# lucian-ilie/SAGE2

Measured on NVIDIA B200. Metric: reads/sec through exact-overlap graph build (SAGE2 steps 1-3), higher is better.
Workload: dtype u64

## Files before the change

sage2_b200/csrc/core.cuh:

```cuda
#pragma once
#include <stdint.h>

#if defined(__CUDACC__)
#define SG_HD __host__ __device__ __forceinline__
#else
#define SG_HD inline
#endif

namespace sg {

typedef uint64_t u64;
typedef uint32_t u32;

constexpr int kMaxWords = 32;
constexpr int kHashThreshold = 100;
constexpr u32 kConnectionsLimit = 300;

SG_HD int words_for_len(int max_len) { return (2 * max_len + 16 + 63) / 64; }
SG_HD int storage_words(int SW) { return SW <= 4 ? 4 : (SW <= 8 ? 8 : (SW <= 16 ? 16 : 32)); }
SG_HD int rec_len(const u64 *rec, int SW) { return (int)(rec[SW - 1] & 0xFFFFull); }
SG_HD int hash_len_for(int min_overlap) { return min_overlap > 64 ? 64 : min_overlap; }

SG_HD u64 window32(const u64 *X, int SW, int s)
{
// ... 26 lines not shown
    return true;
}

SG_HD u64 rev2(u64 w)
{
#if defined(__CUDA_ARCH__)
    w = __brevll(w);
    return ((w >> 1) & 0x5555555555555555ull) | ((w & 0x5555555555555555ull) << 1);
#else
    w = ((w >> 2) & 0x3333333333333333ull) | ((w & 0x3333333333333333ull) << 2);
    w = ((w >> 4) & 0x0F0F0F0F0F0F0F0Full) | ((w & 0x0F0F0F0F0F0F0F0Full) << 4);
    return __builtin_bswap64(w);
#endif
}

SG_HD void revcomp_record(const u64 *F, u64 *R, int SW, int len)
{
    const int sh = 64 * SW - 2 * len;
    const int q = sh >> 6, r = sh & 63;
    for (int w = 0; w < SW; ++w) {
        const int i0 = w + q, i1 = w + q + 1;
        const u64 a = i0 < SW ? rev2(~F[SW - 1 - i0]) : 0ull;
        const u64 b = i1 < SW ? rev2(~F[SW - 1 - i1]) : 0ull;
        R[w] = r == 0 ? a : ((a << r) | (b >> (64 - r)));
    }
    R[SW - 1] |= (u64)len;
}

SG_HD u64 mix64(u64 x)
{
    x ^= x >> 33; x *= 0xff51afd7ed558ccdull; x ^= x >> 33; x *= 0xc4ceb9fe1a85ec53ull; x ^= x >> 33;
    return x;
}
SG_HD u64 hash_key(u64 v0, u64 v1) { return mix64(v1 ^ mix64(v0 + 0x9e3779b97f4a7c15ull)); }
SG_HD u64 mulhi64(u64 a, u64 b)
{
#if defined(__CUDA_ARCH__)
    return __umul64hi(a, b);
#else
    return (u64)(((unsigned __int128)a * b) >> 64);
#endif
// ... 152 lines not shown
```

sage2_b200/csrc/device_utils.cuh:

```cuda
#pragma once
#include <cuda_runtime.h>
#include <stdint.h>
#include <stdio.h>
#include <algorithm>
#include <stdexcept>
#include <string>
#include <vector>

namespace sg {

typedef uint64_t u64;
typedef uint32_t u32;

struct CudaError : public std::runtime_error {
    explicit CudaError(const std::string &m) : std::runtime_error(m) {}
};

#define SG_CUDA(call)                                                                           \
    do {                                                                                        \
        cudaError_t e__ = (call);                                                               \
        if (e__ != cudaSuccess)                                                                 \
            throw sg::CudaError(std::string(#call) + " failed: " + cudaGetErrorString(e__) +    \
                                " at " + __FILE__ + ":" + std::to_string(__LINE__));            \
    } while (0)
// ... 128 lines not shown
{
    cudaStreamSynchronize(st);
    cudaMemPool_t pool;
    if (cudaDeviceGetDefaultMemPool(&pool, device) == cudaSuccess) cudaMemPoolTrimTo(pool, 0);
}

constexpr int kSMs = 148;

inline unsigned long long &launch_counter() { static unsigned long long n = 0; return n; }
#define SG_LAUNCHED()                     \
    do {                                  \
        ++sg::launch_counter();           \
        SG_CUDA(cudaGetLastError());      \
    } while (0)

inline unsigned grid_for(u64 n, unsigned block, unsigned per_thread = 1)
{
    u64 g = (n + (u64)block * per_thread - 1) / ((u64)block * per_thread);
    if (g == 0) g = 1;
    SG_CHECK(g < 0x7FFFFFFFull, "grid too large");
    return (unsigned)g;
}

void exclusive_scan_u32(const u32 *in, u32 *out, u64 n, u32 *d_total, cudaStream_t st);

void reduce_or_and_u64(const u64 *keys, u64 n, u64 *d_or_and, cudaStream_t st);

struct SortCols {
    u64 *a[2];
    u64 *b[2];
// ... 10 lines not shown
```

sage2_b200/csrc/reads.cu:

```cuda
#include <stdlib.h>
#include "context.h"

namespace sg {

constexpr int K1_WARPS = 8;

__global__ void __launch_bounds__(K1_WARPS * 32) max_len_kernel(const int64_t *__restrict__ off, u64 n, int *out)
{
    int m = 0;
    for (u64 i = (u64)blockIdx.x * blockDim.x + threadIdx.x; i < n; i += (u64)gridDim.x * blockDim.x) {
        const int64_t d = off[i + 1] - off[i];
        const int l = d > 0x7FFFFFFF ? 0x7FFFFFFF : (int)d;
        m = l > m ? l : m;
    }
    m = __reduce_max_sync(0xffffffffu, m);
    if ((threadIdx.x & 31) == 0) atomicMax(out, m);
}

__global__ void __launch_bounds__(K1_WARPS * 32) pack_kernel(const uint8_t *__restrict__ bases, const int64_t *__restrict__ off,
                                                              u64 n, int k, int SW, u64 *__restrict__ rec,
                                                              unsigned long long *counters )
{
    __shared__ __align__(16) uint8_t sB[K1_WARPS][32 * kMaxWords];
    __shared__ u64 sF[K1_WARPS][kMaxWords], sR[K1_WARPS][kMaxWords];
// ... 278 lines not shown
    c.cnt.total_bp = h_cnt[1];
    c.cnt.avg_len = h_cnt[0] ? h_cnt[1] / h_cnt[0] : 0;
}

__global__ void iota_kernel(u32 *v, u64 n)
{
    for (u64 i = (u64)blockIdx.x * blockDim.x + threadIdx.x; i < n; i += (u64)gridDim.x * blockDim.x) v[i] = (u32)i;
}

__global__ void gather_word_kernel(const u64 *__restrict__ rec, const u32 *__restrict__ perm, u64 n, int SW, int w, u64 *__restrict__ key)
{
    for (u64 i = (u64)blockIdx.x * blockDim.x + threadIdx.x; i < n; i += (u64)gridDim.x * blockDim.x)
        key[i] = rec[(u64)perm[i] * SW + w];
}

__global__ void unique_flag_kernel(const u64 *__restrict__ rec, const u32 *__restrict__ perm, u64 n_good, int SW, u32 *__restrict__ flag)
{
    for (u64 i = (u64)blockIdx.x * blockDim.x + threadIdx.x; i < n_good; i += (u64)gridDim.x * blockDim.x) {
        u32 f = 1;
        if (i > 0) {
            const u64 *a = rec + (u64)perm[i] * SW, *b = rec + (u64)perm[i - 1] * SW;
            f = 0;
            for (int w = 0; w < SW; ++w) f |= (a[w] != b[w]);
        }
        flag[i] = f;
    }
}

template <bool WITH_RC>
__global__ void unique_write_kernel(const u64 *__restrict__ rec, const u32 *__restrict__ perm, const u32 *__restrict__ flag,
                                    const u32 *__restrict__ uidx, u64 n_good, int SW, int SWS,
                                    u64 *__restrict__ F, u64 *__restrict__ RC, uint16_t *__restrict__ len, u32 *__restrict__ start)
{
    for (u64 i = (u64)blockIdx.x * blockDim.x + threadIdx.x; i < n_good; i += (u64)gridDim.x * blockDim.x) {
        if (!flag[i]) continue;
        const u32 u = uidx[i];
        const u64 *a = rec + (u64)perm[i] * SW;
        u64 f[kMaxWords], r[kMaxWords];
        for (int w = 0; w < SW; ++w) f[w] = a[w];
        const int l = rec_len(f, SW);
        if (WITH_RC) revcomp_record(f, r, SW, l);
        for (int w = 0; w < SWS; ++w) { F[(u64)u * SWS + w] = w < SW ? f[w] : 0ull; if (WITH_RC) RC[(u64)u * SWS + w] = w < SW ? r[w] : 0ull; }
        len[u] = (uint16_t)l;
        start[u] = (u32)i;
    }
}

__global__ void freq_kernel(const u32 *__restrict__ start, u64 U, u64 n_good, uint16_t *__restrict__ freq)
{
    for (u64 u = (u64)blockIdx.x * blockDim.x + threadIdx.x; u < U; u += (u64)gridDim.x * blockDim.x) {
        const u64 e = (u + 1 < U) ? start[u + 1] : n_good;
        freq[u] = (uint16_t)(e - start[u]);
    }
}

static unsigned big_grid(u64 n, unsigned block = 256)
{
    unsigned g = grid_for(n, block, 4);
    return g > kSMs * 16u ? kSMs * 16u : g;
// ... 16 lines not shown
static int sort_skip_bits(u64 n)
{
    int lg = 0;
    while (lg < 63 && (1ull << lg) < n) ++lg;
    int bits = ((lg + 5 + 7) / 8) * 8;
    if (bits < 32) bits = 32;
    if (bits > 48) bits = 48;
    return 64 - bits;
}
__device__ __forceinline__ bool rec_less(const u64 *a, const u64 *b, int SW)
{
    for (int w = 0; w < SW; ++w) { const u64 x = a[w], y = b[w]; if (x != y) return x < y; }
    return false;
}
__global__ void __launch_bounds__(256) tie_fix_kernel(const u64 *__restrict__ rec, const u64 *__restrict__ key, u32 *__restrict__ perm, u64 n, int SW,
                                                        int kSortSkipBits, u32 *__restrict__ overflow)
{
    for (u64 i = (u64)blockIdx.x * blockDim.x + threadIdx.x; i < n; i += (u64)gridDim.x * blockDim.x) {
        const u64 k = key[i] >> kSortSkipBits;
        if ((i > 0 && (key[i - 1] >> kSortSkipBits) == k) || i + 1 >= n || (key[i + 1] >> kSortSkipBits) != k) continue;
        u64 e = i + 2;
        while (e < n && (key[e] >> kSortSkipBits) == k && e - i <= (u64)kTieLimit) ++e;
        if (e - i > (u64)kTieLimit) { *overflow = 1u; continue; }
        for (u64 a = i + 1; a < e; ++a) {
            const u32 x = perm[a];
            const u64 *rx = rec + (u64)x * SW;
            u64 b = a;
            while (b > i && rec_less(rx, rec + (u64)perm[b - 1] * SW, SW)) { perm[b] = perm[b - 1]; --b; }
            perm[b] = x;
        }
    }
}

__global__ void __launch_bounds__(256) run_boundary_kernel(const u64 *__restrict__ key, u64 n, int kSortSkipBits, u32 *__restrict__ flag)
{
    for (u64 i = (u64)blockIdx.x * blockDim.x + threadIdx.x; i < n; i += (u64)gridDim.x * blockDim.x)
        flag[i] = (i == 0 || (key[i] >> kSortSkipBits) != (key[i - 1] >> kSortSkipBits)) ? 1u : 0u;
}
__global__ void __launch_bounds__(256) run_count_kernel(const u32 *__restrict__ flag, const u32 *__restrict__ excl, u64 n, u32 *__restrict__ cnt)
{
    for (u64 i = (u64)blockIdx.x * blockDim.x + threadIdx.x; i < n; i += (u64)gridDim.x * blockDim.x)
        atomicAdd(&cnt[excl[i] + flag[i] - 1], 1u);
}
__global__ void __launch_bounds__(256) run_long_flag_kernel(const u32 *__restrict__ flag, const u32 *__restrict__ excl, const u32 *__restrict__ cnt, u64 n,
                                                            u32 *__restrict__ lflag)
{
    for (u64 i = (u64)blockIdx.x * blockDim.x + threadIdx.x; i < n; i += (u64)gridDim.x * blockDim.x)
        lflag[i] = cnt[excl[i] + flag[i] - 1] > (u32)kTieLimit ? 1u : 0u;
}
__global__ void __launch_bounds__(256) run_compact_kernel(const u32 *__restrict__ lflag, const u32 *__restrict__ lidx, const u32 *__restrict__ flag,
                                                          const u32 *__restrict__ excl, const u32 *__restrict__ perm, u64 n,
                                                          u32 *__restrict__ pos, u32 *__restrict__ val, u64 *__restrict__ run)
{
    for (u64 i = (u64)blockIdx.x * blockDim.x + threadIdx.x; i < n; i += (u64)gridDim.x * blockDim.x)
        if (lflag[i]) { const u32 j = lidx[i]; pos[j] = (u32)i; val[j] = perm[i]; run[j] = (u64)(excl[i] + flag[i] - 1); }
}
__global__ void __launch_bounds__(256) run_scatter_kernel(const u32 *__restrict__ pos, const u32 *__restrict__ val, u64 m, u32 *__restrict__ perm)
{
    for (u64 j = (u64)blockIdx.x * blockDim.x + threadIdx.x; j < m; j += (u64)gridDim.x * blockDim.x) perm[pos[j]] = val[j];
}

static void refine_long_runs(Context &c, const u64 *rec, const u64 *key, u32 *perm, u64 n, int SW, int kSortSkipBits)
{
    cudaStream_t st = c.stream;
    DevBuf<u32> flag(n, st), excl(n, st), cnt(n, st), lflag(n, st), lidx(n, st), d_m(1, st);
    run_boundary_kernel<<<big_grid(n), 256, 0, st>>>(key, n, kSortSkipBits, flag.p);
    SG_LAUNCHED();
    exclusive_scan_u32(flag.p, excl.p, n, nullptr, st);
    SG_CUDA(cudaMemsetAsync(cnt.p, 0, n * sizeof(u32), st));
    run_count_kernel<<<big_grid(n), 256, 0, st>>>(flag.p, excl.p, n, cnt.p);
    SG_LAUNCHED();
    run_long_flag_kernel<<<big_grid(n), 256, 0, st>>>(flag.p, excl.p, cnt.p, n, lflag.p);
    SG_LAUNCHED();
    exclusive_scan_u32(lflag.p, lidx.p, n, d_m.p, st);
    u32 m = 0;
    SG_CUDA(cudaMemcpyAsync(&m, d_m.p, sizeof(u32), cudaMemcpyDeviceToHost, st));
    SG_CUDA(cudaStreamSynchronize(st));
    if (m == 0) return;
    DevBuf<u32> pos(m, st), v0(m, st), v1(m, st);
    DevBuf<u64> a0(m, st), a1(m, st), b0(m, st), b1(m, st);
    run_compact_kernel<<<big_grid(n), 256, 0, st>>>(lflag.p, lidx.p, flag.p, excl.p, perm, n, pos.p, v0.p, b0.p);
    SG_LAUNCHED();
    SortCols cols;
    cols.a[0] = a0.p; cols.a[1] = a1.p; cols.b[0] = b0.p; cols.b[1] = b1.p; cols.v[0] = v0.p; cols.v[1] = v1.p;
    int cur = 0;
    for (int w = SW - 1; w >= 0; --w) {
        gather_word_kernel<<<big_grid(m), 256, 0, st>>>(rec, cols.v[cur], m, SW, w, cols.a[cur]);
        SG_LAUNCHED();
        cur = radix_sort_bits(cols, cur, m, false, 0, w == 0 ? kSortSkipBits : 64, st);
    }
    int id_bits = 1;
    while ((n >> id_bits) != 0) ++id_bits;
    cur = radix_sort_bits(cols, cur, m, true, 0, id_bits, st);
    run_scatter_kernel<<<big_grid(m), 256, 0, st>>>(pos.p, cols.v[cur], m, perm);
    SG_LAUNCHED();
}

constexpr int kSplitBits = 12;
__global__ void __launch_bounds__(256) split_hist_kernel(const u64 *__restrict__ key, u64 n, u32 *__restrict__ hist)
{
    __shared__ u32 sh[1 << kSplitBits];
    for (int b = threadIdx.x; b < (1 << kSplitBits); b += blockDim.x) sh[b] = 0;
    __syncthreads();
    for (u64 i = (u64)blockIdx.x * blockDim.x + threadIdx.x; i < n; i += (u64)gridDim.x * blockDim.x) atomicAdd(&sh[key[i] >> (64 - kSplitBits)], 1u);
    __syncthreads();
    for (int b = threadIdx.x; b < (1 << kSplitBits); b += blockDim.x) if (sh[b]) atomicAdd(&hist[b], sh[b]);
}
__global__ void __launch_bounds__(256) split_flag_kernel(const u64 *__restrict__ key, u64 n, u32 lo_bin, u32 hi_bin, u32 *__restrict__ flag)
{
    for (u64 i = (u64)blockIdx.x * blockDim.x + threadIdx.x; i < n; i += (u64)gridDim.x * blockDim.x) {
        const u32 b = (u32)(key[i] >> (64 - kSplitBits));
        flag[i] = (b >= lo_bin && b < hi_bin) ? 1u : 0u;
    }
}
__global__ void __launch_bounds__(256) split_compact_kernel(const u64 *__restrict__ key, const u32 *__restrict__ val, const u32 *__restrict__ flag,
                                                            const u32 *__restrict__ idx, u64 n, u64 *__restrict__ okey, u32 *__restrict__ oval)
{
    for (u64 i = (u64)blockIdx.x * blockDim.x + threadIdx.x; i < n; i += (u64)gridDim.x * blockDim.x)
        if (flag[i]) { okey[idx[i]] = key[i]; oval[idx[i]] = val[i]; }
}
__global__ void __launch_bounds__(256) revcomp_range_kernel(const u64 *__restrict__ F, u64 *__restrict__ RC, const uint16_t *__restrict__ len,
                                                            u64 lo, u64 hi, int SW, int SWS)
{
    for (u64 u = lo + (u64)blockIdx.x * blockDim.x + threadIdx.x; u < hi; u += (u64)gridDim.x * blockDim.x) {
        u64 f[kMaxWords], r[kMaxWords];
        for (int w = 0; w < SW; ++w) f[w] = F[u * SWS + w];
        revcomp_record(f, r, SW, (int)len[u]);
        for (int w = 0; w < SWS; ++w) RC[u * SWS + w] = w < SW ? r[w] : 0ull;
    }
}

void stage_organize_reads(Context &c, int rank, int world)
{
    cudaStream_t st = c.stream;
    ArenaScope arena_scope(c.arena, st);
    SG_CHECK(world >= 1 && world <= kMaxWorld && rank >= 0 && rank < world, "bad rank / world");
    const u64 n = c.n_input;
    u64 n_good = c.cnt.good_reads;
    const int SW = c.SW;
    c.cnt.unique_reads = 0;
    c.rp_rank = rank; c.rp_world = world; c.rp_local = 0;
    if (n == 0 || n_good == 0) {
        if (world == 1) { c.F.release(); c.RC.release(); c.len.release(); c.freq.release(); }
// ... 35 lines not shown
        u64 n_part = 0;
        for (u32 b = bound[rank]; b < bound[rank + 1]; ++b) n_part += h[b];
        DevBuf<u32> sflag(n_good, st), sidx(n_good, st);
        split_flag_kernel<<<big_grid(n_good), 256, 0, st>>>(ka.p, n_good, bound[rank], bound[rank + 1], sflag.p);
        SG_LAUNCHED();
        exclusive_scan_u32(sflag.p, sidx.p, n_good, nullptr, st);
        split_compact_kernel<<<big_grid(n_good), 256, 0, st>>>(ka.p, va.p, sflag.p, sidx.p, n_good, kb.p, vb.p);
        SG_LAUNCHED();
        cur = 1;
        n_good = n_part;
        if (n_good == 0) return;
    }
    cur = radix_sort_bits(cols, cur, n_good, false, kSortSkipBits, 64, st);
    DevBuf<u32> d_flags(2, st);
    SG_CUDA(cudaMemsetAsync(d_flags.p, 0, 2 * sizeof(u32), st));
    {
        tie_fix_kernel<<<big_grid(n_good), 256, 0, st>>>(rec.p, cols.a[cur], cols.v[cur], n_good, SW, kSortSkipBits, d_flags.p);
        SG_LAUNCHED();
    }
    DevBuf<u32> flag(n_good, st), uidx(n_good, st);
    u32 h_flags[2] = { 0, 0 };
    for (int attempt = 0; attempt < 2; ++attempt) {
        unique_flag_kernel<<<big_grid(n_good), 256, 0, st>>>(rec.p, cols.v[cur], n_good, SW, flag.p);
        SG_LAUNCHED();
        exclusive_scan_u32(flag.p, uidx.p, n_good, d_flags.p + 1, st);
        SG_CUDA(cudaMemcpyAsync(h_flags, d_flags.p, sizeof(h_flags), cudaMemcpyDeviceToHost, st));
        SG_CUDA(cudaStreamSynchronize(st));
        if (!h_flags[0] || attempt == 1) break;
        SG_CUDA(cudaMemsetAsync(d_flags.p, 0, sizeof(u32), st));
        refine_long_runs(c, rec.p, cols.a[cur], cols.v[cur], n_good, SW, kSortSkipBits);
    }
    const u32 *perm = cols.v[cur];
    const u32 U = h_flags[1];
    c.cnt.unique_reads = U;
    c.SWS = storage_words(SW);
    DevBuf<u64> &Fo = world > 1 ? c.F_loc : c.F;
    DevBuf<uint16_t> &lo = world > 1 ? c.len_loc : c.len, &fo = world > 1 ? c.freq_loc : c.freq;
    Fo.alloc((size_t)U * c.SWS, st);
    lo.alloc(U, st);
    fo.alloc(U, st);
    DevBuf<u32> start(U, st);
    if (world > 1) {
        unique_write_kernel<false><<<big_grid(n_good, 128), 128, 0, st>>>(rec.p, perm, flag.p, uidx.p, n_good, SW, c.SWS, Fo.p, nullptr, lo.p, start.p);
    } else {
        c.RC.alloc((size_t)U * c.SWS, st);
        unique_write_kernel<true><<<big_grid(n_good, 128), 128, 0, st>>>(rec.p, perm, flag.p, uidx.p, n_good, SW, c.SWS, Fo.p, c.RC.p, lo.p, start.p);
    }
    SG_LAUNCHED();
    freq_kernel<<<big_grid(U), 256, 0, st>>>(start.p, U, n_good, fo.p);
    SG_LAUNCHED();
    c.rp_local = U;
    c.have_reads = world == 1;
    if (c.opt_low_memory) { SG_CUDA(cudaStreamSynchronize(st)); c.raw.release(); trim_default_pool(c.device, st); }
}

void stage_reads_gather_layout(Context &c, const u64 *counts, void **F, void **len, void **freq, u64 *first, u64 *total)
{
    cudaStream_t st = c.stream;
    SG_CHECK(c.rp_world > 1 && counts != nullptr, "sage2gpu_load_reads_partition must run first");
    SG_CHECK(counts[c.rp_rank] == c.rp_local, "this rank's count does not match its organised reads");
    u64 tot = 0, base = 0;
// ... 9 lines not shown
    SG_CUDA(cudaStreamSynchronize(st));
    c.rp_first = base; c.rp_total = tot;
    if (F) *F = c.F.p;
    if (len) *len = c.len.p;
    if (freq) *freq = c.freq.p;
    if (first) *first = base;
    if (total) *total = tot;
}

void stage_reads_gather_finish(Context &c)
{
    cudaStream_t st = c.stream;
    SG_CHECK(c.rp_world > 1, "sage2gpu_load_reads_partition must run first");
    const u64 U = c.rp_total;
    if (U) {
        revcomp_range_kernel<<<big_grid(U, 128), 128, 0, st>>>(c.F.p, c.RC.p, c.len.p, 0, U, c.SW, c.SWS);
        SG_LAUNCHED();
    }
    c.cnt.unique_reads = U;
    c.have_reads = true;
    if (c.opt_low_memory) { SG_CUDA(cudaStreamSynchronize(st)); c.F_loc.release(); c.len_loc.release(); c.freq_loc.release(); }
}

void stage_raw_gather_layout(Context &c, int rank, int world, const u64 *counts, void **raw, u64 *first, u64 *total)
{
    cudaStream_t st = c.stream;
    SG_CHECK(world >= 1 && world <= kMaxWorld && rank >= 0 && rank < world && counts, "bad rank / world");
    SG_CHECK(counts[rank] == c.n_input, "this rank's count does not match its packed slice");
    u64 tot = 0, base = 0;
    for (int q = 0; q < world; ++q) { if (q < rank) base += counts[q]; tot += counts[q]; }
    SG_CHECK(tot < 0x3FFFFFFFull, "at most 2^30-1 reads");
// ... 22 lines not shown
```

sage2_b200/csrc/table.cu:

```cuda
#include <stdlib.h>
#include "context.h"

namespace sg {

constexpr u64 kCountOne = 1ull << 33;
constexpr u32 kNotOwned = 0xFFFFFFFFu;

__device__ __forceinline__ u64 load_slot(const u64 *p) { return *reinterpret_cast<const volatile u64 *>(p); }

__global__ void __launch_bounds__(256) table_insert_kernel(const u64 *__restrict__ F, const u64 *__restrict__ RC,
                                                            const uint16_t *__restrict__ len, u64 U, int SW, int SWS, int h,
                                                            u64 *__restrict__ slots, u64 nsec, u32 *__restrict__ where,
                                                            int rank, int world, u32 *__restrict__ overflow)
{
    for (u64 t = (u64)blockIdx.x * blockDim.x + threadIdx.x; t < 4 * U; t += (u64)gridDim.x * blockDim.x) {
        const u64 rid = t >> 2;
        const int type = (int)(t & 3);
        u64 v0, v1;
        entry_key(F + rid * SWS, RC + rid * SWS, SW, len[rid], h, type, v0, v1);
        const u64 hsh = hash_key(v0, v1);
        if (key_owner(hsh, world) != rank) { where[t] = kNotOwned; continue; }
        const u64 tag = slot_tag(hsh);
        u64 sec = home_sector(hsh, nsec);
        bool done = false;
// ... 17 lines not shown
                    const u64 old = atomicCAS((unsigned long long *)sp, (unsigned long long)cur, (unsigned long long)(cur + kCountOne));
                    if (old == cur) break;
                    cur = old;
                }
                where[t] = (u32)(kSlotsPerSector * sec + q);
                done = true;
            }
            sec = (sec + 1 == nsec) ? 0 : sec + 1;
            if (++tries > nsec) { *overflow = 1; where[t] = kNotOwned; break; }
        }
    }
}

__global__ void __launch_bounds__(256) table_keys_kernel(const u64 *__restrict__ F, const u64 *__restrict__ RC, const uint16_t *__restrict__ len,
                                                          u64 U, int SW, int SWS, int h, int rank, int world,
                                                          u64 *__restrict__ A, u32 *__restrict__ V, u64 room, unsigned long long *__restrict__ n_out)
{
    __shared__ u32 s_warp[8];
    __shared__ unsigned long long s_base;
    const int lane = threadIdx.x & 31, warp = threadIdx.x >> 5;
    for (u64 r0 = (u64)blockIdx.x * 256; r0 < U; r0 += (u64)gridDim.x * 256) {
        const u64 rid = r0 + threadIdx.x;
        u64 hs[4] = { 0, 0, 0, 0 };
        u32 own = 0;
        if (rid < U) {
            const int l = len[rid];
#pragma unroll
            for (int type = 0; type < 4; ++type) {
                u64 v0, v1;
                entry_key(F + rid * SWS, RC + rid * SWS, SW, l, h, type, v0, v1);
                hs[type] = hash_key(v0, v1);
                if (world <= 1 || key_owner(hs[type], world) == rank) own |= 1u << type;
            }
        }
        if (world <= 1) {
            if (rid < U) {
#pragma unroll
                for (int type = 0; type < 4; ++type) { A[4 * rid + type] = hs[type]; V[4 * rid + type] = (u32)(4 * rid + type); }
            }
            continue;
        }
        const u32 cnt = (u32)__popc(own);
        u32 inc = cnt;
#pragma unroll
        for (int o = 1; o < 32; o <<= 1) { const u32 y = __shfl_up_sync(0xffffffffu, inc, o); if (lane >= o) inc += y; }
        if (lane == 31) s_warp[warp] = inc;
        __syncthreads();
        if (threadIdx.x == 0) {
            u32 tot = 0;
            for (int w = 0; w < 8; ++w) { const u32 x = s_warp[w]; s_warp[w] = tot; tot += x; }
            s_base = tot ? atomicAdd(n_out, (unsigned long long)tot) : 0ull;
        }
        __syncthreads();
        u64 pos = s_base + s_warp[warp] + (inc - cnt);
        if (pos + cnt <= room) {
#pragma unroll
            for (int type = 0; type < 4; ++type)
                if (own & (1u << type)) { A[pos] = hs[type]; V[pos] = (u32)(4 * rid + type); ++pos; }
        }
        __syncthreads();
    }
}

__global__ void __launch_bounds__(256) table_claim_kernel(const u64 *__restrict__ A, const u32 *__restrict__ V, u64 n_rec,
                                                           u64 *__restrict__ slots, u64 nsec, u32 *__restrict__ where,
                                                           u32 *__restrict__ retry, u32 *__restrict__ n_retry)
{
    const u64 i = (u64)blockIdx.x * blockDim.x + threadIdx.x;
    bool again = false;
    if (i < n_rec) {
        const u64 hsh = A[i];
        const u32 t = V[i];
        const u64 tag = slot_tag(hsh);
        const u64 sec = home_sector(hsh, nsec);
        u64 *sp = slots + kSlotsPerSector * sec;
        const ulonglong2 lo = __ldcg(reinterpret_cast<const ulonglong2 *>(sp)), hi = __ldcg(reinterpret_cast<const ulonglong2 *>(sp) + 1);
        const u64 cur[4] = { lo.x, lo.y, hi.x, hi.y };
        int q = -1;
        bool seen = false;
#pragma unroll
        for (int x = 3; x >= 0; --x) {
            if (cur[x] == 0) { q = x; seen = false; }
            else if (slot_get_tag(cur[x]) == tag) seen = true;
        }
        again = true;
        if (q >= 0 && !seen) {
            const u64 old = atomicCAS((unsigned long long *)(sp + q), 0ull, (unsigned long long)slot_encode(hsh, 1, t));
            if (old == 0) { where[i] = (u32)(kSlotsPerSector * sec + q); again = false; }
        }
    }
    __shared__ u32 s_cnt[8];
    const int lane = threadIdx.x & 31, warp = threadIdx.x >> 5;
    const unsigned m = __ballot_sync(0xffffffffu, again);
    if (lane == 0) s_cnt[warp] = (u32)__popc(m);
    __syncthreads();
    u32 base = 0, total = 0;
#pragma unroll
    for (int w = 0; w < 8; ++w) { if (w < warp) base += s_cnt[w]; total += s_cnt[w]; }
    if (again) retry[(u64)blockIdx.x * 256 + base + __popc(m & ((1u << lane) - 1u))] = (u32)i;
    if (threadIdx.x == 0) n_retry[blockIdx.x] = total;
}

__global__ void __launch_bounds__(64) table_insert_sorted_kernel(const u64 *__restrict__ A, const u32 *__restrict__ V, const u32 *__restrict__ retry,
                                                                   const u32 *__restrict__ n_retry,
                                                                   const u64 *__restrict__ F, const u64 *__restrict__ RC,
                                                                   const uint16_t *__restrict__ len, int SW, int SWS, int h,
                                                                   u64 *__restrict__ slots, u64 nsec, u32 *__restrict__ where, u32 *__restrict__ overflow)
{
    const u32 mine = n_retry[blockIdx.x];
    for (u32 k = threadIdx.x; k < mine; k += blockDim.x) {
        const u64 i = retry[(u64)blockIdx.x * 256 + k];
        const u64 hsh = A[i];
        const u32 t = V[i];
        const u64 tag = slot_tag(hsh);
        u64 sec = home_sector(hsh, nsec);
        bool done = false, have_key = false;
        u64 v0 = 0, v1 = 0;
        u64 tries = 0;
        while (!done) {
            for (int q = 0; q < kSlotsPerSector && !done; ++q) {
                u64 *sp = slots + kSlotsPerSector * sec + q;
                u64 cur = load_slot(sp);
                if (cur == 0) {
                    const u64 old = atomicCAS((unsigned long long *)sp, 0ull, (unsigned long long)slot_encode(hsh, 1, t));
                    if (old == 0) { where[i] = (u32)(kSlotsPerSector * sec + q); done = true; break; }
                    cur = old;
                }
                if (slot_get_tag(cur) != tag) continue;
                if (!have_key) { const u64 r1 = t >> 2; entry_key(F + r1 * SWS, RC + r1 * SWS, SW, (t & 1) ? (int)len[r1] : h, h, (int)(t & 3), v0, v1); have_key = true; }
                const u32 rep = (u32)slot_get_payload(cur);
                const u64 r2 = rep >> 2;
                u64 w0, w1;
                entry_key(F + r2 * SWS, RC + r2 * SWS, SW, (rep & 1) ? (int)len[r2] : h, h, (int)(rep & 3), w0, w1);
                if (w0 != v0 || w1 != v1) continue;
                while (slot_get_count(cur) < 127) {
                    const u64 old = atomicCAS((unsigned long long *)sp, (unsigned long long)cur, (unsigned long long)(cur + kCountOne));
                    if (old == cur) break;
                    cur = old;
                }
                where[i] = (u32)(kSlotsPerSector * sec + q);
                done = true;
            }
            sec = (sec + 1 == nsec) ? 0 : sec + 1;
            if (++tries > nsec) { *overflow = 1; where[i] = kNotOwned; break; }
        }
    }
}

__global__ void __launch_bounds__(256) table_fill_sorted_kernel(const u64 *__restrict__ slots, const u32 *__restrict__ where, const u32 *__restrict__ V, u64 n_rec,
                                                                 u32 *__restrict__ cursor, u32 *__restrict__ entries)
{
    for (u64 i = (u64)blockIdx.x * blockDim.x + threadIdx.x; i < n_rec; i += (u64)gridDim.x * blockDim.x) {
        if (where[i] == kNotOwned) continue;
        const u64 v = slots[where[i]];
        const u32 c = slot_get_count(v);
        if (c < 2 || c >= (u32)kHashThreshold) continue;
        const u64 off = slot_get_payload(v);
        entries[off + atomicAdd(&cursor[off], 1u)] = V[i];
    }
}

__global__ void __launch_bounds__(256) table_runs_kernel(const u64 *__restrict__ slots, u64 cap, u32 *__restrict__ run, unsigned long long *counters)
{
    unsigned long long distinct = 0, over = 0;
    for (u64 s = (u64)blockIdx.x * blockDim.x + threadIdx.x; s < cap; s += (u64)gridDim.x * blockDim.x) {
        const u64 v = slots[s];
        const u32 c = v ? slot_get_count(v) : 0u;
        run[s] = (c >= 2 && c < (u32)kHashThreshold) ? c : 0u;
        distinct += v != 0;
        over += c >= (u32)kHashThreshold;
    }
#pragma unroll
    for (int o = 16; o > 0; o >>= 1) { distinct += __shfl_xor_sync(0xffffffffu, distinct, o); over += __shfl_xor_sync(0xffffffffu, over, o); }
    if ((threadIdx.x & 31) == 0) { if (distinct) atomicAdd(&counters[0], distinct); if (over) atomicAdd(&counters[1], over); }
}

__global__ void __launch_bounds__(256) table_offsets_kernel(u64 *__restrict__ slots, u64 cap, const u32 *__restrict__ run, const u32 *__restrict__ off)
{
    for (u64 s = (u64)blockIdx.x * blockDim.x + threadIdx.x; s < cap; s += (u64)gridDim.x * blockDim.x)
        if (run[s]) slots[s] = (slots[s] & ~0x1FFFFFFFFull) | (u64)off[s];
}

__global__ void __launch_bounds__(256) table_fill_kernel(const u64 *__restrict__ slots, const u32 *__restrict__ where, u64 n,
// ... 48 lines not shown

    u64 nsec = (n + n / 2 + kSlotsPerSector - 1) / kSlotsPerSector;
    if (world > 1) nsec = nsec / (u64)world + nsec / (10 * (u64)world) + 1;
    if (nsec < 256) nsec = 256;
    const u64 cap = nsec * kSlotsPerSector;
    SG_CHECK(cap < 0xFFFFFFFFull, "slot index too large for one context");
    c.slots.alloc(c.tb_joint ? cap * (u64)world : cap, st);
    u64 *const slots = c.slots.p + (c.tb_joint ? (u64)rank * cap : 0);
    DevBuf<u32> &entries = c.tb_joint ? c.entries_loc : c.entries;
    SG_CUDA(cudaMemsetAsync(slots, 0, cap * sizeof(u64), st));

    const char *env = getenv("SAGE2GPU_TABLE_BUILD");
    const int forced = !env ? 0 : (env[0] == 'd' ? 1 : 2);
    const bool bucketed = forced ? forced == 2 : (!c.opt_low_memory && cap * sizeof(u64) >= ((size_t)256 << 20));
    DevBuf<u32> where, d_overflow(1, st), v0, v1;
    DevBuf<u64> a0, a1;
    const u32 *recV = nullptr;
    u64 n_rec = n;
    SG_CUDA(cudaMemsetAsync(d_overflow.p, 0, sizeof(u32), st));
    if (!bucketed) {
        where.alloc(n, st);
        table_insert_kernel<<<big_grid(n), 256, 0, st>>>(c.F.p, c.RC.p, c.len.p, U, SW, c.SWS, h, slots, nsec, where.p, rank, world, d_overflow.p);
        SG_LAUNCHED();
    } else {
        u64 room = world > 1 ? n / (u64)world + n / (4 * (u64)world) + 4096 : n;
        if (const char *e = getenv("SAGE2GPU_TABLE_ROOM")) { if (world > 1) room = (u64)atoll(e); }
        DevBuf<unsigned long long> d_nrec(1, st);
        for (;;) {
            a0.alloc(room + 1, st); v0.alloc(room + 1, st);
            SG_CUDA(cudaMemsetAsync(d_nrec.p, 0, sizeof(unsigned long long), st));
            table_keys_kernel<<<big_grid(U), 256, 0, st>>>(c.F.p, c.RC.p, c.len.p, U, SW, c.SWS, h, rank, world, a0.p, v0.p, room, d_nrec.p);
            SG_LAUNCHED();
            if (world <= 1) break;
            unsigned long long h_nrec = 0;
            SG_CUDA(cudaMemcpyAsync(&h_nrec, d_nrec.p, sizeof(h_nrec), cudaMemcpyDeviceToHost, st));
            SG_CUDA(cudaStreamSynchronize(st));
            n_rec = h_nrec;
            if (n_rec <= room) break;
            room = n_rec;
        }
        a1.alloc(n_rec + 1, st); v1.alloc(n_rec + 1, st);
        SortCols cols;
        cols.a[0] = a0.p; cols.a[1] = a1.p; cols.b[0] = cols.b[1] = nullptr; cols.v[0] = v0.p; cols.v[1] = v1.p;
        const int cur = radix_sort_bits(cols, 0, n_rec, false, 56, 64, st);
        recV = cols.v[cur];
        where.alloc(n_rec + 1, st);
        if (n_rec) {
            const unsigned blocks = grid_for(n_rec, 256);
            DevBuf<u32> retry((u64)blocks * 256, st), n_retry(blocks, st);
            table_claim_kernel<<<blocks, 256, 0, st>>>(cols.a[cur], recV, n_rec, slots, nsec, where.p, retry.p, n_retry.p);
            SG_LAUNCHED();
            table_insert_sorted_kernel<<<blocks, 64, 0, st>>>(cols.a[cur], recV, retry.p, n_retry.p, c.F.p, c.RC.p, c.len.p, SW, c.SWS, h, slots, nsec,
                                                               where.p, d_overflow.p);
            SG_LAUNCHED();
        }
    }

    DevBuf<u32> run(cap, st), off(cap, st), d_total(1, st);
    DevBuf<unsigned long long> d_cnt(2, st);
    SG_CUDA(cudaMemsetAsync(d_cnt.p, 0, 2 * sizeof(unsigned long long), st));
    table_runs_kernel<<<big_grid(cap), 256, 0, st>>>(slots, cap, run.p, d_cnt.p);
    SG_LAUNCHED();
    exclusive_scan_u32(run.p, off.p, cap, d_total.p, st);
    u32 M = 0;
    unsigned long long h_cnt[2];
    u32 h_overflow = 0;
    SG_CUDA(cudaMemcpyAsync(&h_overflow, d_overflow.p, sizeof(u32), cudaMemcpyDeviceToHost, st));
    SG_CUDA(cudaMemcpyAsync(&M, d_total.p, sizeof(u32), cudaMemcpyDeviceToHost, st));
    SG_CUDA(cudaMemcpyAsync(h_cnt, d_cnt.p, sizeof(h_cnt), cudaMemcpyDeviceToHost, st));
    SG_CUDA(cudaStreamSynchronize(st));
    SG_CHECK(h_overflow == 0, "slot index of this table shard is full (key split too uneven)");

    entries.alloc(M, st);
    c.tb_entries = M;
    if (M) {
        table_offsets_kernel<<<big_grid(cap), 256, 0, st>>>(slots, cap, run.p, off.p);
// ... 70 lines not shown
```

Baseline: 182.1 million.

## Fuse dedupe flags into tie fix, group-parallel unique write, carry keys through table sort

Dedupe flags are now computed inside tie_fix_kernel and refine_long_runs, which removes the separate unique_flag pass and its retry loop with an extra host sync. unique_write and revcomp kernels now assign one group of threads per record, share the record through shared memory, and use 256-bit vector loads and stores, with reverse-complement computed per word. The bucketed table build sorts the first key word alongside the hash, so collision checks in insert compare sorted arrays instead of re-extracting keys from F/RC. Slot payloads temporarily hold sorted indices and are remapped in table_runs. Optional stats printing is also added.

Measured after the change: 189.9 million, median of 6. 1.04x the previous value.

```diff
diff --git a/sage2_b200/csrc/core.cuh b/sage2_b200/csrc/core.cuh
--- a/sage2_b200/csrc/core.cuh
+++ b/sage2_b200/csrc/core.cuh
@@ -64,17 +64,19 @@
 #endif
 }
 
-SG_HD void revcomp_record(const u64 *F, u64 *R, int SW, int len)
+SG_HD u64 revcomp_word(const u64 *F, int SW, int len, int w)
 {
     const int sh = 64 * SW - 2 * len;
     const int q = sh >> 6, r = sh & 63;
-    for (int w = 0; w < SW; ++w) {
-        const int i0 = w + q, i1 = w + q + 1;
-        const u64 a = i0 < SW ? rev2(~F[SW - 1 - i0]) : 0ull;
-        const u64 b = i1 < SW ? rev2(~F[SW - 1 - i1]) : 0ull;
-        R[w] = r == 0 ? a : ((a << r) | (b >> (64 - r)));
-    }
-    R[SW - 1] |= (u64)len;
+    const int i0 = w + q, i1 = w + q + 1;
+    const u64 a = i0 < SW ? rev2(~F[SW - 1 - i0]) : 0ull;
+    const u64 b = i1 < SW ? rev2(~F[SW - 1 - i1]) : 0ull;
+    const u64 x = r == 0 ? a : ((a << r) | (b >> (64 - r)));
+    return w == SW - 1 ? x | (u64)len : x;
+}
+SG_HD void revcomp_record(const u64 *F, u64 *R, int SW, int len)
+{
+    for (int w = 0; w < SW; ++w) R[w] = revcomp_word(F, SW, len, w);
 }
 
 SG_HD u64 mix64(u64 x)
diff --git a/sage2_b200/csrc/device_utils.cuh b/sage2_b200/csrc/device_utils.cuh
--- a/sage2_b200/csrc/device_utils.cuh
+++ b/sage2_b200/csrc/device_utils.cuh
@@ -2,6 +2,7 @@
 #include <cuda_runtime.h>
 #include <stdint.h>
 #include <stdio.h>
+#include <stdlib.h>
 #include <algorithm>
 #include <stdexcept>
 #include <string>
@@ -166,6 +167,8 @@
         SG_CUDA(cudaGetLastError());      \
     } while (0)
 
+inline bool stage_stats_enabled() { return getenv("SAGE2GPU_STAGE_STATS") != nullptr; }
+
 inline unsigned grid_for(u64 n, unsigned block, unsigned per_thread = 1)
 {
     u64 g = (n + (u64)block * per_thread - 1) / ((u64)block * per_thread);
diff --git a/sage2_b200/csrc/reads.cu b/sage2_b200/csrc/reads.cu
--- a/sage2_b200/csrc/reads.cu
+++ b/sage2_b200/csrc/reads.cu
@@ -316,35 +316,60 @@
         key[i] = rec[(u64)perm[i] * SW + w];
 }
 
-__global__ void unique_flag_kernel(const u64 *__restrict__ rec, const u32 *__restrict__ perm, u64 n_good, int SW, u32 *__restrict__ flag)
-{
-    for (u64 i = (u64)blockIdx.x * blockDim.x + threadIdx.x; i < n_good; i += (u64)gridDim.x * blockDim.x) {
-        u32 f = 1;
-        if (i > 0) {
-            const u64 *a = rec + (u64)perm[i] * SW, *b = rec + (u64)perm[i - 1] * SW;
-            f = 0;
-            for (int w = 0; w < SW; ++w) f |= (a[w] != b[w]);
-        }
-        flag[i] = f;
-    }
-}
-
+__device__ __forceinline__ bool rec_differs(const u64 *a, const u64 *b, int SW)
+{
+    u64 d = 0;
+    for (int w = 0; w < SW; ++w) d |= a[w] ^ b[w];
+    return d != 0;
+}
+
+constexpr int UW_THREADS = 256;
+__device__ __forceinline__ void ld256(const u64 *p, u64 (&v)[4])
+{
+    asm volatile("ld.global.nc.v4.u64 {%0,%1,%2,%3}, [%4];" : "=l"(v[0]), "=l"(v[1]), "=l"(v[2]), "=l"(v[3]) : "l"(p));
+}
+__device__ __forceinline__ void st256(u64 *p, const u64 (&v)[4])
+{
+    asm volatile("st.global.v4.u64 [%0], {%1,%2,%3,%4};" :: "l"(p), "l"(v[0]), "l"(v[1]), "l"(v[2]), "l"(v[3]) : "memory");
+}
 template <bool WITH_RC>
-__global__ void unique_write_kernel(const u64 *__restrict__ rec, const u32 *__restrict__ perm, const u32 *__restrict__ flag,
-                                    const u32 *__restrict__ uidx, u64 n_good, int SW, int SWS,
-                                    u64 *__restrict__ F, u64 *__restrict__ RC, uint16_t *__restrict__ len, u32 *__restrict__ start)
-{
-    for (u64 i = (u64)blockIdx.x * blockDim.x + threadIdx.x; i < n_good; i += (u64)gridDim.x * blockDim.x) {
-        if (!flag[i]) continue;
-        const u32 u = uidx[i];
-        const u64 *a = rec + (u64)perm[i] * SW;
-        u64 f[kMaxWords], r[kMaxWords];
-        for (int w = 0; w < SW; ++w) f[w] = a[w];
-        const int l = rec_len(f, SW);
-        if (WITH_RC) revcomp_record(f, r, SW, l);
-        for (int w = 0; w < SWS; ++w) { F[(u64)u * SWS + w] = w < SW ? f[w] : 0ull; if (WITH_RC) RC[(u64)u * SWS + w] = w < SW ? r[w] : 0ull; }
-        len[u] = (uint16_t)l;
-        start[u] = (u32)i;
+__device__ __forceinline__ void store_group_words(const u64 *grp, const u64 (&f)[4], int g, int SW, int len, u64 *Fdst, u64 *RCdst)
+{
+    st256(Fdst + 4 * g, f);
+    if (WITH_RC) {
+        u64 r[4];
+#pragma unroll
+        for (int j = 0; j < 4; ++j) { const int w = 4 * g + j; r[j] = w < SW ? revcomp_word(grp, SW, len, w) : 0ull; }
+        st256(RCdst + 4 * g, r);
+    }
+}
+
+template <bool WITH_RC>
+__global__ void __launch_bounds__(UW_THREADS) unique_write_kernel(const u64 *__restrict__ rec, const u32 *__restrict__ perm, const u32 *__restrict__ flag,
+                                                                   const u32 *__restrict__ uidx, u64 n_good, int SW, int SWS,
+                                                                   u64 *__restrict__ F, u64 *__restrict__ RC, uint16_t *__restrict__ len, u32 *__restrict__ start)
+{
+    __shared__ u64 sRec[UW_THREADS * 4];
+    const int G = SWS / 4, g = threadIdx.x & (G - 1);
+    const u64 per_block = UW_THREADS / G;
+    u64 *grp = sRec + 4 * (threadIdx.x - g);
+    for (u64 i0 = (u64)blockIdx.x * per_block; i0 < n_good; i0 += (u64)gridDim.x * per_block) {
+        const u64 i = i0 + threadIdx.x / G;
+        const bool active = i < n_good && flag[i];
+        u64 f[4] = { 0, 0, 0, 0 };
+        if (active) {
+            const u64 *a = rec + (u64)perm[i] * SW;
+#pragma unroll
+            for (int j = 0; j < 4; ++j) { const int w = 4 * g + j; if (w < SW) f[j] = a[w]; grp[4 * g + j] = f[j]; }
+        }
+        __syncwarp();
+        if (active) {
+            const u32 u = uidx[i];
+            const int l = rec_len(grp, SW);
+            store_group_words<WITH_RC>(grp, f, g, SW, l, F + (u64)u * SWS, WITH_RC ? RC + (u64)u * SWS : nullptr);
+            if (g == 0) { len[u] = (uint16_t)l; start[u] = (u32)i; }
+        }
+        __syncwarp();
     }
 }
 
@@ -391,11 +416,13 @@
     return false;
 }
 __global__ void __launch_bounds__(256) tie_fix_kernel(const u64 *__restrict__ rec, const u64 *__restrict__ key, u32 *__restrict__ perm, u64 n, int SW,
-                                                        int kSortSkipBits, u32 *__restrict__ overflow)
+                                                        int kSortSkipBits, u32 *__restrict__ flag, u32 *__restrict__ overflow)
 {
     for (u64 i = (u64)blockIdx.x * blockDim.x + threadIdx.x; i < n; i += (u64)gridDim.x * blockDim.x) {
         const u64 k = key[i] >> kSortSkipBits;
-        if ((i > 0 && (key[i - 1] >> kSortSkipBits) == k) || i + 1 >= n || (key[i + 1] >> kSortSkipBits) != k) continue;
+        if (i > 0 && (key[i - 1] >> kSortSkipBits) == k) continue;
+        flag[i] = 1u;
+        if (i + 1 >= n || (key[i + 1] >> kSortSkipBits) != k) continue;
         u64 e = i + 2;
         while (e < n && (key[e] >> kSortSkipBits) == k && e - i <= (u64)kTieLimit) ++e;
         if (e - i > (u64)kTieLimit) { *overflow = 1u; continue; }
@@ -406,6 +433,7 @@
             while (b > i && rec_less(rx, rec + (u64)perm[b - 1] * SW, SW)) { perm[b] = perm[b - 1]; --b; }
             perm[b] = x;
         }
+        for (u64 a = i + 1; a < e; ++a) flag[a] = rec_differs(rec + (u64)perm[a] * SW, rec + (u64)perm[a - 1] * SW, SW) ? 1u : 0u;
     }
 }
 
@@ -436,27 +464,35 @@
 {
     for (u64 j = (u64)blockIdx.x * blockDim.x + threadIdx.x; j < m; j += (u64)gridDim.x * blockDim.x) perm[pos[j]] = val[j];
 }
-
-static void refine_long_runs(Context &c, const u64 *rec, const u64 *key, u32 *perm, u64 n, int SW, int kSortSkipBits)
+__global__ void __launch_bounds__(256) run_member_flag_kernel(const u64 *__restrict__ rec, const u32 *__restrict__ pos, const u32 *__restrict__ bound,
+                                                              const u32 *__restrict__ perm, u64 m, int SW, u32 *__restrict__ flag)
+{
+    for (u64 j = (u64)blockIdx.x * blockDim.x + threadIdx.x; j < m; j += (u64)gridDim.x * blockDim.x) {
+        const u32 i = pos[j];
+        if (!bound[i]) flag[i] = rec_differs(rec + (u64)perm[i] * SW, rec + (u64)perm[i - 1] * SW, SW) ? 1u : 0u;
+    }
+}
+
+static u32 refine_long_runs(Context &c, const u64 *rec, const u64 *key, u32 *perm, u64 n, int SW, int kSortSkipBits, u32 *dedupe_flag)
 {
     cudaStream_t st = c.stream;
-    DevBuf<u32> flag(n, st), excl(n, st), cnt(n, st), lflag(n, st), lidx(n, st), d_m(1, st);
-    run_boundary_kernel<<<big_grid(n), 256, 0, st>>>(key, n, kSortSkipBits, flag.p);
-    SG_LAUNCHED();
-    exclusive_scan_u32(flag.p, excl.p, n, nullptr, st);
+    DevBuf<u32> bound(n, st), excl(n, st), cnt(n, st), lflag(n, st), lidx(n, st), d_m(1, st);
+    run_boundary_kernel<<<big_grid(n), 256, 0, st>>>(key, n, kSortSkipBits, bound.p);
+    SG_LAUNCHED();
+    exclusive_scan_u32(bound.p, excl.p, n, nullptr, st);
     SG_CUDA(cudaMemsetAsync(cnt.p, 0, n * sizeof(u32), st));
-    run_count_kernel<<<big_grid(n), 256, 0, st>>>(flag.p, excl.p, n, cnt.p);
-    SG_LAUNCHED();
-    run_long_flag_kernel<<<big_grid(n), 256, 0, st>>>(flag.p, excl.p, cnt.p, n, lflag.p);
+    run_count_kernel<<<big_grid(n), 256, 0, st>>>(bound.p, excl.p, n, cnt.p);
+    SG_LAUNCHED();
+    run_long_flag_kernel<<<big_grid(n), 256, 0, st>>>(bound.p, excl.p, cnt.p, n, lflag.p);
     SG_LAUNCHED();
     exclusive_scan_u32(lflag.p, lidx.p, n, d_m.p, st);
     u32 m = 0;
     SG_CUDA(cudaMemcpyAsync(&m, d_m.p, sizeof(u32), cudaMemcpyDeviceToHost, st));
     SG_CUDA(cudaStreamSynchronize(st));
-    if (m == 0) return;
+    if (m == 0) return 0;
     DevBuf<u32> pos(m, st), v0(m, st), v1(m, st);
     DevBuf<u64> a0(m, st), a1(m, st), b0(m, st), b1(m, st);
-    run_compact_kernel<<<big_grid(n), 256, 0, st>>>(lflag.p, lidx.p, flag.p, excl.p, perm, n, pos.p, v0.p, b0.p);
+    run_compact_kernel<<<big_grid(n), 256, 0, st>>>(lflag.p, lidx.p, bound.p, excl.p, perm, n, pos.p, v0.p, b0.p);
     SG_LAUNCHED();
     SortCols cols;
     cols.a[0] = a0.p; cols.a[1] = a1.p; cols.b[0] = b0.p; cols.b[1] = b1.p; cols.v[0] = v0.p; cols.v[1] = v1.p;
@@ -471,6 +507,9 @@
     cur = radix_sort_bits(cols, cur, m, true, 0, id_bits, st);
     run_scatter_kernel<<<big_grid(m), 256, 0, st>>>(pos.p, cols.v[cur], m, perm);
     SG_LAUNCHED();
+    run_member_flag_kernel<<<big_grid(m), 256, 0, st>>>(rec, pos.p, bound.p, perm, m, SW, dedupe_flag);
+    SG_LAUNCHED();
+    return m;
 }
 
 constexpr int kSplitBits = 12;
@@ -496,14 +535,29 @@
     for (u64 i = (u64)blockIdx.x * blockDim.x + threadIdx.x; i < n; i += (u64)gridDim.x * blockDim.x)
         if (flag[i]) { okey[idx[i]] = key[i]; oval[idx[i]] = val[i]; }
 }
-__global__ void __launch_bounds__(256) revcomp_range_kernel(const u64 *__restrict__ F, u64 *__restrict__ RC, const uint16_t *__restrict__ len,
-                                                            u64 lo, u64 hi, int SW, int SWS)
-{
-    for (u64 u = lo + (u64)blockIdx.x * blockDim.x + threadIdx.x; u < hi; u += (u64)gridDim.x * blockDim.x) {
-        u64 f[kMaxWords], r[kMaxWords];
-        for (int w = 0; w < SW; ++w) f[w] = F[u * SWS + w];
-        revcomp_record(f, r, SW, (int)len[u]);
-        for (int w = 0; w < SWS; ++w) RC[u * SWS + w] = w < SW ? r[w] : 0ull;
+__global__ void __launch_bounds__(UW_THREADS) revcomp_range_kernel(const u64 *__restrict__ F, u64 *__restrict__ RC, const uint16_t *__restrict__ len,
+                                                                   u64 U, int SW, int SWS)
+{
+    __shared__ u64 sRec[UW_THREADS * 4];
+    const int G = SWS / 4, g = threadIdx.x & (G - 1);
+    const u64 per_block = UW_THREADS / G;
+    u64 *grp = sRec + 4 * (threadIdx.x - g);
+    for (u64 u0 = (u64)blockIdx.x * per_block; u0 < U; u0 += (u64)gridDim.x * per_block) {
+        const u64 u = u0 + threadIdx.x / G;
+        u64 f[4] = { 0, 0, 0, 0 };
+        if (u < U) {
+            ld256(F + u * SWS + 4 * g, f);
+#pragma unroll
+            for (int j = 0; j < 4; ++j) grp[4 * g + j] = f[j];
+        }
+        __syncwarp();
+        if (u < U) {
+            u64 r[4];
+#pragma unroll
+            for (int j = 0; j < 4; ++j) { const int w = 4 * g + j; r[j] = w < SW ? revcomp_word(grp, SW, (int)len[u], w) : 0ull; }
+            st256(RC + u * SWS + 4 * g, r);
+        }
+        __syncwarp();
     }
 }
 
@@ -569,22 +623,19 @@
     cur = radix_sort_bits(cols, cur, n_good, false, kSortSkipBits, 64, st);
     DevBuf<u32> d_flags(2, st);
     SG_CUDA(cudaMemsetAsync(d_flags.p, 0, 2 * sizeof(u32), st));
-    {
-        tie_fix_kernel<<<big_grid(n_good), 256, 0, st>>>(rec.p, cols.a[cur], cols.v[cur], n_good, SW, kSortSkipBits, d_flags.p);
-        SG_LAUNCHED();
-    }
     DevBuf<u32> flag(n_good, st), uidx(n_good, st);
+    tie_fix_kernel<<<big_grid(n_good), 256, 0, st>>>(rec.p, cols.a[cur], cols.v[cur], n_good, SW, kSortSkipBits, flag.p, d_flags.p);
+    SG_LAUNCHED();
     u32 h_flags[2] = { 0, 0 };
-    for (int attempt = 0; attempt < 2; ++attempt) {
-        unique_flag_kernel<<<big_grid(n_good), 256, 0, st>>>(rec.p, cols.v[cur], n_good, SW, flag.p);
-        SG_LAUNCHED();
-        exclusive_scan_u32(flag.p, uidx.p, n_good, d_flags.p + 1, st);
-        SG_CUDA(cudaMemcpyAsync(h_flags, d_flags.p, sizeof(h_flags), cudaMemcpyDeviceToHost, st));
-        SG_CUDA(cudaStreamSynchronize(st));
-        if (!h_flags[0] || attempt == 1) break;
-        SG_CUDA(cudaMemsetAsync(d_flags.p, 0, sizeof(u32), st));
-        refine_long_runs(c, rec.p, cols.a[cur], cols.v[cur], n_good, SW, kSortSkipBits);
-    }
+    SG_CUDA(cudaMemcpyAsync(h_flags, d_flags.p, sizeof(u32), cudaMemcpyDeviceToHost, st));
+    SG_CUDA(cudaStreamSynchronize(st));
+    u32 m_long = 0;
+    if (h_flags[0]) m_long = refine_long_runs(c, rec.p, cols.a[cur], cols.v[cur], n_good, SW, kSortSkipBits, flag.p);
+    exclusive_scan_u32(flag.p, uidx.p, n_good, d_flags.p + 1, st);
+    SG_CUDA(cudaMemcpyAsync(h_flags + 1, d_flags.p + 1, sizeof(u32), cudaMemcpyDeviceToHost, st));
+    SG_CUDA(cudaStreamSynchronize(st));
+    if (stage_stats_enabled())
+        fprintf(stderr, "sage2gpu stats: organize_reads reads=%llu long_run_members=%u unique=%u\n", (unsigned long long)n_good, m_long, h_flags[1]);
     const u32 *perm = cols.v[cur];
     const u32 U = h_flags[1];
     c.cnt.unique_reads = U;
@@ -595,11 +646,12 @@
     lo.alloc(U, st);
     fo.alloc(U, st);
     DevBuf<u32> start(U, st);
+    const unsigned uw_grid = big_grid(n_good * (c.SWS / 4), UW_THREADS);
     if (world > 1) {
-        unique_write_kernel<false><<<big_grid(n_good, 128), 128, 0, st>>>(rec.p, perm, flag.p, uidx.p, n_good, SW, c.SWS, Fo.p, nullptr, lo.p, start.p);
+        unique_write_kernel<false><<<uw_grid, UW_THREADS, 0, st>>>(rec.p, perm, flag.p, uidx.p, n_good, SW, c.SWS, Fo.p, nullptr, lo.p, start.p);
     } else {
         c.RC.alloc((size_t)U * c.SWS, st);
-        unique_write_kernel<true><<<big_grid(n_good, 128), 128, 0, st>>>(rec.p, perm, flag.p, uidx.p, n_good, SW, c.SWS, Fo.p, c.RC.p, lo.p, start.p);
+        unique_write_kernel<true><<<uw_grid, UW_THREADS, 0, st>>>(rec.p, perm, flag.p, uidx.p, n_good, SW, c.SWS, Fo.p, c.RC.p, lo.p, start.p);
     }
     SG_LAUNCHED();
     freq_kernel<<<big_grid(U), 256, 0, st>>>(start.p, U, n_good, fo.p);
@@ -639,7 +691,7 @@
     SG_CHECK(c.rp_world > 1, "sage2gpu_load_reads_partition must run first");
     const u64 U = c.rp_total;
     if (U) {
-        revcomp_range_kernel<<<big_grid(U, 128), 128, 0, st>>>(c.F.p, c.RC.p, c.len.p, 0, U, c.SW, c.SWS);
+        revcomp_range_kernel<<<big_grid(U * (c.SWS / 4), UW_THREADS), UW_THREADS, 0, st>>>(c.F.p, c.RC.p, c.len.p, U, c.SW, c.SWS);
         SG_LAUNCHED();
     }
     c.cnt.unique_reads = U;
diff --git a/sage2_b200/csrc/table.cu b/sage2_b200/csrc/table.cu
--- a/sage2_b200/csrc/table.cu
+++ b/sage2_b200/csrc/table.cu
@@ -55,29 +55,33 @@
 
 __global__ void __launch_bounds__(256) table_keys_kernel(const u64 *__restrict__ F, const u64 *__restrict__ RC, const uint16_t *__restrict__ len,
                                                           u64 U, int SW, int SWS, int h, int rank, int world,
-                                                          u64 *__restrict__ A, u32 *__restrict__ V, u64 room, unsigned long long *__restrict__ n_out)
+                                                          u64 *__restrict__ A, u64 *__restrict__ B, u32 *__restrict__ V, u64 room,
+                                                          unsigned long long *__restrict__ n_out)
 {
     __shared__ u32 s_warp[8];
     __shared__ unsigned long long s_base;
     const int lane = threadIdx.x & 31, warp = threadIdx.x >> 5;
     for (u64 r0 = (u64)blockIdx.x * 256; r0 < U; r0 += (u64)gridDim.x * 256) {
         const u64 rid = r0 + threadIdx.x;
-        u64 hs[4] = { 0, 0, 0, 0 };
+        u64 hs[4] = { 0, 0, 0, 0 }, ks[4] = { 0, 0, 0, 0 };
         u32 own = 0;
         if (rid < U) {
             const int l = len[rid];
 #pragma unroll
             for (int type = 0; type < 4; ++type) {
-                u64 v0, v1;
-                entry_key(F + rid * SWS, RC + rid * SWS, SW, l, h, type, v0, v1);
-                hs[type] = hash_key(v0, v1);
+                u64 v1;
+                entry_key(F + rid * SWS, RC + rid * SWS, SW, l, h, type, ks[type], v1);
+                hs[type] = hash_key(ks[type], v1);
                 if (world <= 1 || key_owner(hs[type], world) == rank) own |= 1u << type;
             }
         }
         if (world <= 1) {
             if (rid < U) {
 #pragma unroll
-                for (int type = 0; type < 4; ++type) { A[4 * rid + type] = hs[type]; V[4 * rid + type] = (u32)(4 * rid + type); }
+                for (int type = 0; type < 4; ++type) {
+                    A[4 * rid + type] = hs[type]; V[4 * rid + type] = (u32)(4 * rid + type);
+                    if (B) B[4 * rid + type] = ks[type];
+                }
             }
             continue;
         }
@@ -97,13 +101,13 @@
         if (pos + cnt <= room) {
 #pragma unroll
             for (int type = 0; type < 4; ++type)
-                if (own & (1u << type)) { A[pos] = hs[type]; V[pos] = (u32)(4 * rid + type); ++pos; }
+                if (own & (1u << type)) { A[pos] = hs[type]; V[pos] = (u32)(4 * rid + type); if (B) B[pos] = ks[type]; ++pos; }
         }
         __syncthreads();
     }
 }
 
-__global__ void __launch_bounds__(256) table_claim_kernel(const u64 *__restrict__ A, const u32 *__restrict__ V, u64 n_rec,
+__global__ void __launch_bounds__(256) table_claim_kernel(const u64 *__restrict__ A, u64 n_rec,
                                                            u64 *__restrict__ slots, u64 nsec, u32 *__restrict__ where,
                                                            u32 *__restrict__ retry, u32 *__restrict__ n_retry)
 {
@@ -111,7 +115,6 @@
     bool again = false;
     if (i < n_rec) {
         const u64 hsh = A[i];
-        const u32 t = V[i];
         const u64 tag = slot_tag(hsh);
         const u64 sec = home_sector(hsh, nsec);
         u64 *sp = slots + kSlotsPerSector * sec;
@@ -126,7 +129,7 @@
         }
         again = true;
         if (q >= 0 && !seen) {
-            const u64 old = atomicCAS((unsigned long long *)(sp + q), 0ull, (unsigned long long)slot_encode(hsh, 1, t));
+            const u64 old = atomicCAS((unsigned long long *)(sp + q), 0ull, (unsigned long long)slot_encode(hsh, 1, i));
             if (old == 0) { where[i] = (u32)(kSlotsPerSector * sec + q); again = false; }
         }
     }
@@ -142,38 +145,31 @@
     if (threadIdx.x == 0) n_retry[blockIdx.x] = total;
 }
 
-__global__ void __launch_bounds__(64) table_insert_sorted_kernel(const u64 *__restrict__ A, const u32 *__restrict__ V, const u32 *__restrict__ retry,
+__global__ void __launch_bounds__(64) table_insert_sorted_kernel(const u64 *__restrict__ A, const u64 *__restrict__ B, const u32 *__restrict__ retry,
                                                                    const u32 *__restrict__ n_retry,
-                                                                   const u64 *__restrict__ F, const u64 *__restrict__ RC,
-                                                                   const uint16_t *__restrict__ len, int SW, int SWS, int h,
                                                                    u64 *__restrict__ slots, u64 nsec, u32 *__restrict__ where, u32 *__restrict__ overflow)
 {
     const u32 mine = n_retry[blockIdx.x];
     for (u32 k = threadIdx.x; k < mine; k += blockDim.x) {
         const u64 i = retry[(u64)blockIdx.x * 256 + k];
         const u64 hsh = A[i];
-        const u32 t = V[i];
+        const u64 v0 = B ? B[i] : 0ull;
         const u64 tag = slot_tag(hsh);
         u64 sec = home_sector(hsh, nsec);
-        bool done = false, have_key = false;
-        u64 v0 = 0, v1 = 0;
+        bool done = false;
         u64 tries = 0;
         while (!done) {
             for (int q = 0; q < kSlotsPerSector && !done; ++q) {
                 u64 *sp = slots + kSlotsPerSector * sec + q;
                 u64 cur = load_slot(sp);
                 if (cur == 0) {
-                    const u64 old = atomicCAS((unsigned long long *)sp, 0ull, (unsigned long long)slot_encode(hsh, 1, t));
+                    const u64 old = atomicCAS((unsigned long long *)sp, 0ull, (unsigned long long)slot_encode(hsh, 1, i));
                     if (old == 0) { where[i] = (u32)(kSlotsPerSector * sec + q); done = true; break; }
                     cur = old;
                 }
                 if (slot_get_tag(cur) != tag) continue;
-                if (!have_key) { const u64 r1 = t >> 2; entry_key(F + r1 * SWS, RC + r1 * SWS, SW, (t & 1) ? (int)len[r1] : h, h, (int)(t & 3), v0, v1); have_key = true; }
-                const u32 rep = (u32)slot_get_payload(cur);
-                const u64 r2 = rep >> 2;
-                u64 w0, w1;
-                entry_key(F + r2 * SWS, RC + r2 * SWS, SW, (rep & 1) ? (int)len[r2] : h, h, (int)(rep & 3), w0, w1);
-                if (w0 != v0 || w1 != v1) continue;
+                const u64 rep = slot_get_payload(cur);
+                if (A[rep] != hsh || (B && B[rep] != v0)) continue;
                 while (slot_get_count(cur) < 127) {
                     const u64 old = atomicCAS((unsigned long long *)sp, (unsigned long long)cur, (unsigned long long)(cur + kCountOne));
                     if (old == cur) break;
@@ -201,13 +197,16 @@
     }
 }
 
-__global__ void __launch_bounds__(256) table_runs_kernel(const u64 *__restrict__ slots, u64 cap, u32 *__restrict__ run, unsigned long long *counters)
+__global__ void __launch_bounds__(256) table_runs_kernel(u64 *__restrict__ slots, u64 cap, const u32 *__restrict__ recV, u32 *__restrict__ run,
+                                                          unsigned long long *counters)
 {
     unsigned long long distinct = 0, over = 0;
     for (u64 s = (u64)blockIdx.x * blockDim.x + threadIdx.x; s < cap; s += (u64)gridDim.x * blockDim.x) {
         const u64 v = slots[s];
         const u32 c = v ? slot_get_count(v) : 0u;
-        run[s] = (c >= 2 && c < (u32)kHashThreshold) ? c : 0u;
+        const bool has_run = c >= 2 && c < (u32)kHashThreshold;
+        run[s] = has_run ? c : 0u;
+        if (recV && v && !has_run) slots[s] = (v & ~0x1FFFFFFFFull) | (u64)recV[slot_get_payload(v)];
         distinct += v != 0;
         over += c >= (u32)kHashThreshold;
     }
@@ -286,7 +285,8 @@
     const int forced = !env ? 0 : (env[0] == 'd' ? 1 : 2);
     const bool bucketed = forced ? forced == 2 : (!c.opt_low_memory && cap * sizeof(u64) >= ((size_t)256 << 20));
     DevBuf<u32> where, d_overflow(1, st), v0, v1;
-    DevBuf<u64> a0, a1;
+    DevBuf<u64> a0, a1, b0, b1;
+    const bool with_v0 = h > 32;
     const u32 *recV = nullptr;
     u64 n_rec = n;
     SG_CUDA(cudaMemsetAsync(d_overflow.p, 0, sizeof(u32), st));
@@ -300,8 +300,9 @@
         DevBuf<unsigned long long> d_nrec(1, st);
         for (;;) {
             a0.alloc(room + 1, st); v0.alloc(room + 1, st);
+            if (with_v0) b0.alloc(room + 1, st);
             SG_CUDA(cudaMemsetAsync(d_nrec.p, 0, sizeof(unsigned long long), st));
-            table_keys_kernel<<<big_grid(U), 256, 0, st>>>(c.F.p, c.RC.p, c.len.p, U, SW, c.SWS, h, rank, world, a0.p, v0.p, room, d_nrec.p);
+            table_keys_kernel<<<big_grid(U), 256, 0, st>>>(c.F.p, c.RC.p, c.len.p, U, SW, c.SWS, h, rank, world, a0.p, b0.p, v0.p, room, d_nrec.p);
             SG_LAUNCHED();
             if (world <= 1) break;
             unsigned long long h_nrec = 0;
@@ -312,26 +313,34 @@
             room = n_rec;
         }
         a1.alloc(n_rec + 1, st); v1.alloc(n_rec + 1, st);
+        if (with_v0) b1.alloc(n_rec + 1, st);
         SortCols cols;
-        cols.a[0] = a0.p; cols.a[1] = a1.p; cols.b[0] = cols.b[1] = nullptr; cols.v[0] = v0.p; cols.v[1] = v1.p;
+        cols.a[0] = a0.p; cols.a[1] = a1.p; cols.b[0] = b0.p; cols.b[1] = b1.p; cols.v[0] = v0.p; cols.v[1] = v1.p;
         const int cur = radix_sort_bits(cols, 0, n_rec, false, 56, 64, st);
         recV = cols.v[cur];
         where.alloc(n_rec + 1, st);
         if (n_rec) {
             const unsigned blocks = grid_for(n_rec, 256);
             DevBuf<u32> retry((u64)blocks * 256, st), n_retry(blocks, st);
-            table_claim_kernel<<<blocks, 256, 0, st>>>(cols.a[cur], recV, n_rec, slots, nsec, where.p, retry.p, n_retry.p);
+            table_claim_kernel<<<blocks, 256, 0, st>>>(cols.a[cur], n_rec, slots, nsec, where.p, retry.p, n_retry.p);
             SG_LAUNCHED();
-            table_insert_sorted_kernel<<<blocks, 64, 0, st>>>(cols.a[cur], recV, retry.p, n_retry.p, c.F.p, c.RC.p, c.len.p, SW, c.SWS, h, slots, nsec,
-                                                               where.p, d_overflow.p);
+            table_insert_sorted_kernel<<<blocks, 64, 0, st>>>(cols.a[cur], cols.b[cur], retry.p, n_retry.p, slots, nsec, where.p, d_overflow.p);
             SG_LAUNCHED();
+            if (stage_stats_enabled()) {
+                std::vector<u32> h_retry(blocks);
+                SG_CUDA(cudaMemcpyAsync(h_retry.data(), n_retry.p, blocks * sizeof(u32), cudaMemcpyDeviceToHost, st));
+                SG_CUDA(cudaStreamSynchronize(st));
+                u64 tot = 0;
+                for (u32 x : h_retry) tot += x;
+                fprintf(stderr, "sage2gpu stats: build_table records=%llu retry_records=%llu\n", (unsigned long long)n_rec, (unsigned long long)tot);
+            }
         }
     }
 
     DevBuf<u32> run(cap, st), off(cap, st), d_total(1, st);
     DevBuf<unsigned long long> d_cnt(2, st);
     SG_CUDA(cudaMemsetAsync(d_cnt.p, 0, 2 * sizeof(unsigned long long), st));
-    table_runs_kernel<<<big_grid(cap), 256, 0, st>>>(slots, cap, run.p, d_cnt.p);
+    table_runs_kernel<<<big_grid(cap), 256, 0, st>>>(slots, cap, recV, run.p, d_cnt.p);
     SG_LAUNCHED();
     exclusive_scan_u32(run.p, off.p, cap, d_total.p, st);
     u32 M = 0;
```
